# Shiakaron/Iterative-solvers-summer-2020

Hardware: AMD Instinct MI355X
Metric: Newton-steps/sec + JVP SpMV HBM GB/s (% peak), 4096^2 grid, 1/2/4/8 GPU (higher is better)
Workload: dtype f64

## Files before the change

include/nkhip.h:

```cpp
#ifndef NKHIP_H
#define NKHIP_H

#include <stdint.h>

#ifdef __cplusplus
extern "C" {
#endif

#define NK_OK 0
#define NK_NO_CONVERGENCE 1
#define NK_NONFINITE 2
#define NK_ZERO_STEP 3
#define NK_BAD_RHS 4
#define NK_EINVAL (-1)
#define NK_EHIP (-2)
#define NK_ECOMM (-3)
#define NK_ENOMEM (-4)

#define NKHIP_ABI_VERSION 3

#define NK_JVP_FD 0
#define NK_JVP_ANALYTIC 1

typedef struct nk_opts {
// ... 55 lines not shown
                int64_t ny, int64_t nx, double h, double r, double k, double g, double zs,
                double sc, void* stream);

int nk_sh_arnoldi_fused(const double* const* V_dev, const double* coef, int32_t nv,
                        const double* w_dev, double tau, const double* x0_dev, const double* G0_dev,
                        const double* z_dev, int64_t ny, int64_t nx, double h, double r, double k,
                        double g, double zs, double sc, double* v_out_dev, double* w_out_dev,
                        double* dots, void* stream);

int64_t nk_edge_elems(int64_t ny, int64_t nx);
int nk_edge_gather(const double* v_dev, double* E_dev, int64_t ny, int64_t nx, void* stream);
int nk_sh_arnoldi_fused_edges(const double* const* V_dev, const double* const* E_dev,
                              const double* coef, int32_t nv, const double* w_dev, double tau,
                              const double* x0_dev, const double* G0_dev, const double* z_dev,
                              int64_t ny, int64_t nx, double h, double r, double k, double g,
                              double zs, double sc, double* v_out_dev, double* w_out_dev,
                              double* Ev_out_dev, double* Ew_out_dev, double* dots, void* stream);
int64_t nk_arnoldi_mbox_launches(void);

int nk_dot(const double* x_dev, const double* y_dev, int64_t n, double* out, void* stream);
int nk_nrm2(const double* x_dev, int64_t n, double* out, void* stream);
int nk_maxnorm(const double* x_dev, int64_t n, double* out, void* stream);
int nk_axpy(double a, const double* x_dev, double* y_dev, int64_t n, void* stream);
int nk_scal(double a, double* x_dev, int64_t n, void* stream);
int nk_mdot(const double* const* V_dev, int32_t m, const double* w_dev, int64_t n, double* out,
            void* stream);
int nk_maxpy(const double* const* V_dev, const double* coef, int32_t m, double* y_dev, int64_t n,
             void* stream);

int nk_stream_copy(const double* src_dev, double* dst_dev, int64_t n, void* stream);

int nk_debug_bounds(int64_t* violations, int32_t* first_line, int32_t reset);
int nk_debug_mailbox(int64_t* counts, int32_t reset);
int nk_debug_ctl_step(int32_t form, int32_t t, const int32_t* ints, const double* scal,
                      const double* sig, const double* h, const double* cs, const double* sn,
                      const double* gram, const double* red, void* state_out, void* mirror_out,
                      double* prm_out, uint32_t* status_out);

int nk_comm_unique_id_bytes(void);
int nk_comm_get_unique_id(void* out);
int nk_comm_create_rccl(nk_comm** out, const void* unique_id, int32_t rank, int32_t nranks);
int nk_comm_create_loopback(nk_comm** out, int32_t nranks);
int nk_comm_peer_handle_bytes(void);
int nk_comm_create_peer(nk_comm** out, int32_t rank, int32_t nranks, int64_t max_nx,
                        void* handle_out);
int nk_comm_peer_connect(nk_comm* c, const void* handles);
int nk_comm_destroy(nk_comm* c);
int nk_comm_abort(nk_comm* c);
int nk_comm_selftest(nk_comm* c, int64_t nx, void* stream);
int nk_comm_selftest_push(nk_comm* c, int64_t nx, void* stream);

int nk_sh_create(nk_sh** out, int64_t ny_local, int64_t nx, int64_t ny_global, double h, double r,
                 double k, double g, const nk_opts* opts, nk_comm* comm, void* stream);
int nk_sh_destroy(nk_sh* s);
int nk_sh_step(nk_sh* s, const double* u_prev_dev, double* u_next_dev, nk_stats* stats);
int nk_sh_set_opts(nk_sh* s, const nk_opts* opts);
int nk_sh_kernel_profile(nk_sh* s, nk_kprof* out, int32_t max);
int nk_sh_reset_profile(nk_sh* s);
int nk_sh_step_log(nk_sh* s, double* steps, int32_t max);
int64_t nk_sh_workspace_bytes(nk_sh* s);

typedef int (*nk_residual_fn)(void* ctx, const double* x_dev, double* f_dev, int64_t n);
int64_t nk_solve_workspace_bytes(int64_t n, const nk_opts* opts);
int nk_solve(nk_residual_fn F, void* ctx, const double* x0_dev, double* x_dev, int64_t n,
             const nk_opts* opts, nk_stats* stats, void* stream, void* workspace,
             int64_t workspace_bytes);
// ... 64 lines not shown
```

iterative-solvers-summer-2020_amd/csrc/capi.cpp:

```cpp
#include <hip/hip_runtime.h>

#include <cmath>
#include <cstdlib>
#include <cstdio>
#include <cstring>
#include <mutex>
#include <memory>
#include <new>
#include <vector>

#include "../../include/nkhip.h"
#include "comm.h"
#include "nk_kernels.h"
#include "nk_solver.h"
#include "droplet_problem.h"
#include "mems_problem.h"
#include "sh_problem.h"
#include "shlin.h"

using namespace nk;

namespace {

hipStream_t S(void* s) { return static_cast<hipStream_t>(s); }
// ... 305 lines not shown
  const int rc = reduce_call(n, nv, nv, nv, res, S(stream), [&](double* part, int64_t* nb) {
    return mdot_launch(w, nullptr, P, m, n, part, S(stream), nb);
  });
  for (int i = 0; i < m; ++i) out[i] = res[i];
  return rc;
}

int nk_maxpy(const double* const* V, const double* coef, int32_t m, double* y, int64_t n,
             void* stream) {
  if (!V || !coef || !y || m < 0 || m > kMaxVec || n < 0) return NK_EINVAL;
  VecList P;
  for (int i = 0; i < m; ++i) {
    P.p[i] = V[i];
    P.c[i] = coef[i];
  }
  int64_t nb = 0;
  return hip_rc(combo_launch(y, y, 1.0, P, m, n, nullptr, S(stream), &nb));
}

int nk_stream_copy(const double* src, double* dst, int64_t n, void* stream) {
  if (!src || !dst || n < 0) return NK_EINVAL;
  return hip_rc(stream_copy_launch(src, dst, n, S(stream)));
}

int nk_debug_bounds(int64_t* violations, int32_t* first_line, int32_t reset) {
  const int rc = arnoldi_check_counters(violations, first_line, reset != 0);
  return rc == 0 ? NK_OK : (rc == -1 ? NK_EINVAL : NK_EHIP);
}

int nk_debug_mailbox(int64_t* counts, int32_t reset) {
  if (!counts) return NK_EINVAL;
  const int rc = arnoldi_mailbox_counters(counts, reset != 0);
  return rc == 0 ? NK_OK : (rc == -1 ? NK_EINVAL : NK_EHIP);
}

int nk_debug_ctl_step(int32_t form, int32_t t, const int32_t* ints, const double* scal,
                      const double* sig, const double* h, const double* cs, const double* sn,
                      const double* gram, const double* red, void* state_out, void* mirror_out,
                      double* prm_out, uint32_t* status_out) {
  if (!state_out) return int(sizeof(ArnCtlState));
  if ((form != 0 && form != 1) || t < 1 || t + 1 > kArnMaxNV || !ints || !scal || !sig || !h ||
      !cs || !sn || !gram || !red || !mirror_out || !prm_out || !status_out)
    return NK_EINVAL;
  const int nval = 2 * (t + 1) + 1;
  ArnCtlState *hS = nullptr, *dS = nullptr;
  uint32_t* status = nullptr;
  double *prm = nullptr, *dred = nullptr;
  hipError_t e = hipHostMalloc(reinterpret_cast<void**>(&hS), sizeof(ArnCtlState), 0);
  if (e == hipSuccess)
    e = hipHostMalloc(reinterpret_cast<void**>(&status), sizeof(uint32_t) * (kMaxVec + 2), 0);
  if (e == hipSuccess) e = hipMalloc(reinterpret_cast<void**>(&dS), sizeof(ArnCtlState));
  if (e == hipSuccess) e = hipMalloc(reinterpret_cast<void**>(&prm), sizeof(double) * kCtlPrm);
  if (e == hipSuccess) e = hipMalloc(reinterpret_cast<void**>(&dred), sizeof(double) * 2 * nval);
  if (e == hipSuccess) {
    std::memset(hS, 0, sizeof(ArnCtlState));
    std::memset(status, 0, sizeof(uint32_t) * (kMaxVec + 2));
    ArnCtlState& S = *hS;
    S.j = ints[0];
    S.hn_pending = ints[1];
    S.m = ints[2];
    S.nv_max = ints[3];
    S.halt = ints[4];
    S.steps = ints[5];
    S.wnorm[t - 1] = scal[0];
    S.gv[t - 1] = scal[1];
    S.sig_est[t] = scal[2];
// ... 508 lines not shown
```

iterative-solvers-summer-2020_amd/csrc/krylov.hip:

```cpp
#include <cmath>
#include <cstdlib>

#include "nk_device.h"
#include "nk_kernels.h"

namespace nk {
namespace {

constexpr int BS = kKrylovBlock;
constexpr int PAIRS = kKrylovPerThread / 2;

template <bool VEC>
__device__ __forceinline__ double2 ld2(const double* p, int64_t i, int64_t n) {
  if (VEC && i + 1 < n) return *reinterpret_cast<const double2*>(p + i);
  double2 r;
  r.x = (i < n) ? p[i] : 0.0;
  r.y = (i + 1 < n) ? p[i + 1] : 0.0;
  return r;
}

typedef double dv2 __attribute__((ext_vector_type(2)));
template <bool VEC, bool NT>
__device__ __forceinline__ double2 ld2s(const double* p, int64_t i, int64_t n) {
  if (NT && VEC && i + 1 < n) {
// ... 149 lines not shown
    if (eo.E) {
      const uint32_t nx = uint32_t(eo.nx), ny = uint32_t(eo.ny);
      uint32_t q = uint32_t(base) / nx, c = uint32_t(base) - q * nx;
#pragma unroll
      for (int k = 0; k < PAIRS; ++k) {
        if (base + k * 2 * BS < n) {
          const dv2 ev = {acc[k].x, acc[k].y};
          if (c % kEdgeW == 0)
            reinterpret_cast<dv2*>(eo.E)[2 * ((c / kEdgeW) * ny + q) + 1] = ev;
          if ((c + 2) % kEdgeW == 0 || c + 2 == nx)
            reinterpret_cast<dv2*>(eo.E)[2 * ((c + 2 == nx ? 0 : (c + 2) / kEdgeW) * ny + q)] = ev;
        }
        for (c += 2 * BS; c >= nx; c -= nx) ++q;
      }
    }
#pragma unroll
    for (int k = 0; k < PAIRS; ++k) {
      st2<VEC>(out, base + k * 2 * BS, n, acc[k]);
      const int64_t i = base + k * 2 * BS;
      if (i < n) {
        red[0] += acc[k].x * acc[k].x;
        red[1] = nmax(red[1], fabs(acc[k].x));
      }
      if (i + 1 < n) {
        red[0] += acc[k].y * acc[k].y;
        red[1] = nmax(red[1], fabs(acc[k].y));
      }
    }
  }
  if (partial) {
    const double v = block_reduce<2, 1, BS>(red);
    if (threadIdx.x < 2) partial[int64_t(threadIdx.x) * nblk + grp] = v;
  }
}

constexpr int RB = 1024;

__global__ void __launch_bounds__(RB) reduce_final_kernel(const double* partial, int64_t nblk,
                                                          int nsum, double* result,
                                                          double* result_host) {
  const int k = blockIdx.x;
  const double s = reduce_column<RB>(partial + int64_t(k) * nblk, nblk, k < nsum);
  if (threadIdx.x == 0) {
    result[k] = s;
    if (result_host) result_host[k] = s;
  }
}

template <bool VEC>
__global__ void __launch_bounds__(256) axpby_kernel(double a, const double* x, double b,
                                                    const double* y, double* out, int64_t n) {
  const int64_t i = 2 * (int64_t(blockIdx.x) * 256 + threadIdx.x);
  if (i >= n) return;
  const double2 xv = ld2<VEC>(x, i, n);
  double2 r = make_double2(a * xv.x, a * xv.y);
  if (y) {
    const double2 yv = ld2<VEC>(y, i, n);
    r.x += b * yv.x;
    r.y += b * yv.y;
  }
  st2<VEC>(out, i, n, r);
}

__global__ void __launch_bounds__(256) fddiff_kernel(double* w, const double* f0, double sc,
                                                     int64_t n) {
  const int64_t i = int64_t(blockIdx.x) * 256 + threadIdx.x;
// ... 100 lines not shown
  if (nb <= kSmallChunks) {
    if (vec)
      hipLaunchKernelGGL((combo_kernel<true, false, 8>), grid, block, 0, s, out, in, cin, P, np, n,
                         cpb, partial, rev, prm, eo);
    else
      hipLaunchKernelGGL((combo_kernel<false, false, 8>), grid, block, 0, s, out, in, cin, P, np,
                         n, cpb, partial, rev, prm, eo);
  } else if (vec && nt) {
    hipLaunchKernelGGL((combo_kernel<true, true, 2>), grid, block, 0, s, out, in, cin, P, np, n,
                       cpb, partial, rev, prm, eo);
  } else if (vec) {
    hipLaunchKernelGGL((combo_kernel<true, false, 2>), grid, block, 0, s, out, in, cin, P, np, n,
                       cpb, partial, rev, prm, eo);
  } else {
    hipLaunchKernelGGL((combo_kernel<false, false, 2>), grid, block, 0, s, out, in, cin, P, np, n,
                       cpb, partial, rev, prm, eo);
  }
  return hipGetLastError();
}
}

hipError_t combo_launch(double* out, const double* in, double cin, const VecList& P, int np,
                        int64_t n, double* partial, hipStream_t s, int64_t* nblk,
                        const EdgeOut& eo) {
  return combo_any(out, in, cin, P, np, n, partial, s, nblk, nullptr, eo);
}

hipError_t combo_prm_launch(double* out, const double* in, const double* prm, const VecList& P,
                            int np, int64_t n, hipStream_t s) {
  if (!prm || np > kArnMaxNV) return hipErrorInvalidValue;
  return combo_any(out, in, 0.0, P, np, n, nullptr, s, nullptr, prm, EdgeOut{});
}

hipError_t reduce_final_launch(const double* partial, int64_t nblk, int nsum, int nv,
                               double* result, double* result_host, hipStream_t s) {
  if (nv <= 0) return hipSuccess;
  hipLaunchKernelGGL(reduce_final_kernel, dim3(unsigned(nv)), dim3(RB), 0, s, partial, nblk, nsum,
                     result, result_host);
  return hipGetLastError();
}

namespace {
typedef double sdv2 __attribute__((ext_vector_type(2)));
__global__ void __launch_bounds__(256) stream_copy_kernel(const sdv2* __restrict__ src,
                                                          sdv2* __restrict__ dst, int64_t n2) {
  const int64_t base = int64_t(blockIdx.x) * 1024 + threadIdx.x;
  sdv2 v[4];
#pragma unroll
  for (int k = 0; k < 4; ++k) {
    const int64_t i = base + k * 256;
    if (i < n2) v[k] = __builtin_nontemporal_load(src + i);
  }
#pragma unroll
  for (int k = 0; k < 4; ++k) {
    const int64_t i = base + k * 256;
    if (i < n2) __builtin_nontemporal_store(v[k], dst + i);
  }
}

}

hipError_t stream_copy_launch(const double* src, double* dst, int64_t n, hipStream_t s) {
  if (n <= 0) return hipSuccess;
  if (!al16(src) || !al16(dst) || n % 2) return hipErrorInvalidValue;
  const int64_t n2 = n / 2;
  hipLaunchKernelGGL(stream_copy_kernel, dim3(unsigned((n2 + 1023) / 1024)), dim3(256), 0, s,
// ... 49 lines not shown
```

iterative-solvers-summer-2020_amd/csrc/lgmres.cpp:

```cpp
#include <algorithm>
#include <atomic>
#include <cstddef>
#include <cfloat>
#include <cmath>
#include <cstdlib>
#include <cstring>

#include "nk_solver.h"
#include "peer_dev.h"

namespace nk {

namespace {
constexpr double kEps = DBL_EPSILON;
constexpr double kLagMinRatio2 = 1e-12;

bool devctl_enabled(bool multi) {
  const char* v = std::getenv("NKHIP_DEVCTL");
  if (v && v[0] == '0') return false;
  if (v && v[0] == '1') return true;
  return multi;
}

bool lag_enabled() {
  static const bool on = [] {
    const char* v = std::getenv("NKHIP_LAGNORM");
    return !(v && v[0] == '0');
  }();
  return on;
}
}

int NewtonKrylov::issue_step(int j, const double* z, double zs, double znorm, bool dev_scale,
                             bool have_w) {
  const int64_t n = E_.n;
  zp_[j] = z;
  hS_->zs[j] = zs;
  double* w = V_[j + 1];
  int rc;
  if (have_w) {
    rc = NK_OK;
    st_->njvp += 1;
  } else if (dev_scale) {
    rc = P_.jvp_dev(X_, G0_, z, E_.dres(Engine::kSlotCombo), omega_, w);
    st_->njvp += 1;
  } else if (znorm == 0.0) {
    rc = E_.launch(K_COPY, 8.0 * n,
                   [&] { return hipMemsetAsync(w, 0, sizeof(double) * n, E_.s); });
    if (!rc) rc = P_.publish_edges(w);
  } else {
    rc = P_.jvp(X_, G0_, z, zs, omega_ / znorm, w);
    st_->njvp += 1;
  }
  if (rc) return rc;
  st_->n_arnoldi += 1;
  VecList P;
  for (int i = 0; i <= j; ++i) P.p[i] = V_[i];
  int64_t nblk = 0;
  const double* g = (j > 0) ? V_[j] : nullptr;
  rc = E_.launch(K_MDOT, 8.0 * n * (j + 2),
                 [&] { return mdot_launch(w, g, P, j + 1, n, E_.partial(), E_.s, &nblk); });
  if (rc) return rc;
// ... 23 lines not shown
  ArnCtlState& S = *hS_;
  S.m = m;
  S.halt = 0;
  S.steps = 0;
  S.ptol = ptol;
  S.omega = omega_;
  S.lag_ratio2 = kLagMinRatio2;
  double* const sig = S.sig;
  double* const rn = S.rn;
  double* const sig_est = S.sig_est;
  double* const wnorm = S.wnorm;
  double* const zs_ = S.zs;
  double* const h = S.h;
  sig[0] = 1.0 / b_norm;
  rn[0] = b_norm;
  double hcur[kMaxVec + 2];
  double red[2 * kMaxVec + 2];
  for (int i = 0; i < kMaxVec + 2; ++i) S.gv[i] = 0.0;
  S.gv[0] = 1.0;

  auto input = [&](int j, const double** z, double* zs, double* zn) {
    if (j < n_o) {
      const int slot = (ohead_ + j) % K;
      *z = outer_[slot];
      *zs = osig_[slot];
      *zn = osig_[slot] * orn_[slot];
    } else {
      *z = V_[j > n_o ? j : 0];
      const int q = j > n_o ? j : 0;
      *zs = sig[q];
      *zn = sig[q] * rn[q];
    }
  };
  auto finish = [&](int i, double hn) -> bool {
    for (int k = 0; k <= i; ++k) hcur[k] = h[k];
    hcur[i + 1] = hn;
    const double alpha = 1.0 / hn;
    sig[i + 1] = std::isfinite(alpha) ? alpha : 1.0;
    rn[i + 1] = hn;
    const bool breakdown = !(hn > kEps * wnorm[i]);
    for (int k = 0; k < i; ++k) {
      const double t = S.cs[k] * hcur[k] + S.sn[k] * hcur[k + 1];
      hcur[k + 1] = -S.sn[k] * hcur[k] + S.cs[k] * hcur[k + 1];
      hcur[k] = t;
    }
    detail::givens(hcur[i], hcur[i + 1], &S.cs[i], &S.sn[i]);
    hcur[i] = S.cs[i] * hcur[i] + S.sn[i] * hcur[i + 1];
    for (int k = 0; k <= i; ++k) S.R[k][i] = hcur[k];
    S.gv[i + 1] = -S.sn[i] * S.gv[i];
    S.gv[i] = S.cs[i] * S.gv[i];
    return std::fabs(S.gv[i + 1]) < ptol || breakdown;
  };

  int rc;
  {
    const double* z;
    double zs, zn;
    input(0, &z, &zs, &zn);
    const bool have = spec_.valid && n_o > 0 && z == spec_.z && zs == spec_.zs &&
                      zn == spec_.zn && V_[1] == spec_.w && X_ == spec_.x && G0_ == spec_.g;
    spec_.valid = false;
    rc = issue_step(0, z, zs, zn, false, have);
  }
  sig_est[0] = 0.0;
  if (!rc) rc = E_.sync();
  if (rc) return rc;
  int j = 0, last = 0;
  bool hn_pending = false;
  for (;;) {
    const int np = j + 1;
    std::memcpy(red, E_.hres(Engine::slot_mdot(j)), sizeof(double) * (2 * np + 1));
    double tau = 1.0;
    if (hn_pending) {
      hn_pending = false;
      if (finish(j - 1, std::sqrt(red[np + j]))) {
        st_->njvp -= 1;
        st_->n_arnoldi -= 1;
        last = j - 1;
        break;
      }
      if (sig_est[j] > 0.0) {
        tau = sig[j] / sig_est[j];
        zs_[j] = sig[j];
      }
    }
    const double ww = tau * tau * red[2 * np];
    if (!std::isfinite(ww)) return NK_NONFINITE;
    wnorm[j] = std::sqrt(ww);
    for (int i = 0; i < j; ++i) S.gram[j][i] = sig[j] * sig[i] * red[np + i];
    double hh = 0.0;
    for (int i = 0; i <= j; ++i) {
      double acc = tau * sig[i] * red[i];
      for (int k = 0; k < i; ++k) acc -= S.gram[i][k] * h[k];
      h[i] = acc;
      hh += acc * acc;
    }
    VecList U;
    for (int i = 0; i <= j; ++i) {
      U.p[i] = V_[i];
      U.c[i] = -h[i] * sig[i];
    }
    double* w = V_[j + 1];
    const bool more = j + 1 < m;
    const bool next_is_v = more && (j + 1 > n_o);
    const double est = ww - hh;
    const bool lag_step = more && lag && (!next_is_v || est > kLagMinRatio2 * ww);
    int64_t nblk = 0;
    if (lag_step && P_.has_fused(j + 1)) {
      const double* z = nullptr;
      double zs, zn;
      if (next_is_v) {
        const double e = std::sqrt(est);
        zs = 1.0 / e;
        zn = zs * e;
      } else {
        input(j + 1, &z, &zs, &zn);
      }
      if (zn != 0.0) {
        const double* Vp[kMaxVec];
        double cc[kMaxVec];
        for (int i = 0; i <= j; ++i) {
          Vp[i] = V_[i];
          cc[i] = U.c[i];
        }
        int64_t nw = 0;
        double* vout = Sv_;
        rc = P_.fused_step(Vp, cc, j + 1, w, tau, X_, G0_, z, zs, omega_ / zn, vout, V_[j + 2],
                           &nw, nullptr);
        if (rc) return rc;
        Sv_ = V_[j + 1];
        V_[j + 1] = vout;
        zp_[j + 1] = next_is_v ? vout : z;
        zs_[j + 1] = zs;
        sig_est[j + 1] = next_is_v ? zs : 0.0;
        st_->njvp += 1;
        st_->n_arnoldi += 1;
        const int np1 = j + 2;
        rc = E_.reduce_async(nw, 2 * np1 + 1, 2 * np1 + 1, Engine::slot_mdot(j + 1));
        if (rc) return rc;
        hn_pending = true;
// ... 62 lines not shown
    rc = E_.sync();
    if (rc) return rc;
    const bool stop = finish(j, std::sqrt(E_.hres(Engine::kSlotCombo)[0]));
    if (spec) zs_[j + 1] = sig[j + 1];
    if (stop || !more) {
      if (spec) {
        st_->njvp -= 1;
        st_->n_arnoldi -= 1;
      }
      last = j;
      break;
    }
    if (!spec) {
      const double* z;
      double zs, zn;
      input(j + 1, &z, &zs, &zn);
      rc = issue_step(j + 1, z, zs, zn, false);
      if (!rc) rc = E_.sync();
      if (rc) return rc;
    }
    sig_est[j + 1] = 0.0;
    ++j;
  }
  j = last;
  if (!std::isfinite(S.R[j][j])) return NK_OK;
  double y[kMaxVec + 1];
  detail::lstsq_upper(S.R, j + 1, S.gv, y);
  for (int i = 0; i <= j; ++i) {
    y[i] *= b_norm;
    if (!std::isfinite(y[i])) return NK_OK;
  }
  const int slot = (o_.outer_k > 0 && ocount_ < o_.outer_k) ? (ohead_ + ocount_) % K : ohead_;
  VecList Z;
  for (int i = 0; i <= j; ++i) {
    Z.p[i] = zp_[i];
    Z.c[i] = y[i] * zs_[i];
  }
  int64_t nblk = 0;
  double* d = outer_[slot];
  const EdgeOut eo = P_.edge_out(d);
  rc = E_.launch(K_COMBO, 8.0 * n * (j + 2), [&] {
    return combo_launch(d, nullptr, 0.0, Z, j + 1, n, E_.partial(), E_.s, &nblk, eo);
  });
  if (!rc) rc = P_.publish_edges(d, eo.E != nullptr);
  if (rc) return rc;
  double r2[2];
  rc = E_.reduce(nblk, 1, 2, r2);
  if (rc) return rc;
  const double nx = std::sqrt(r2[0]);
  if (nx > 0 && o_.outer_k > 0) {
    osig_[slot] = 1.0 / nx;
    orn_[slot] = nx;
    if (ocount_ < o_.outer_k)
      ++ocount_;
    else
      ohead_ = (ohead_ + 1) % K;
  }
  *dnorm = nx;
  *dmax = r2[1];
  *dvec = d;
  return NK_OK;
}

int NewtonKrylov::device_steps() {
  ArnCtlState& S = *hS_;
  const int t0 = S.j;
  int nvmax = t0;
  while (nvmax + 1 < S.m && nvmax + 1 <= kArnMaxNV &&
         (P_.has_fused(nvmax + 1) || P_.has_jvp_prm()))
    ++nvmax;
  if (nvmax < t0 + 1) return E_.wait_results(Engine::slot_mdot(t0), 2 * (t0 + 1) + 1);
  S.nv_max = nvmax;
  S.halt = 0;
  S.steps = 0;
  S.arrive = 0;
// ... 159 lines not shown
```

iterative-solvers-summer-2020_amd/csrc/nk_kernels.h:

```cpp
#pragma once

#include <hip/hip_runtime.h>

#include <cstdint>

#include "peer_dev.h"

struct nk_comm;

namespace nk {

bool peer_fuse_enabled();
bool slab_x_enabled(const nk_comm* c);
uint64_t device_wait_ticks();
double device_wait_seconds();

struct Field {
  const double* base;
  const double* lo;
  const double* hi;
};

inline Field periodic(const double* p) { return Field{p, nullptr, nullptr}; }

// ... 44 lines not shown
  bool nt_p0 = false;
};

bool traversal_reverse();

hipError_t stencil_launch(SMode m, const StencilArgs& a, hipStream_t s, int64_t* nblk);
int64_t stencil_partial_slots(int64_t ny, int64_t nx);
double stencil_bytes_per_point(SMode m, bool has_xt);

constexpr int kMaxVec = 64;
struct VecList {
  const double* p[kMaxVec];
  double c[kMaxVec];
};

constexpr int kKrylovBlock = 256;
constexpr int kKrylovPerThread = 8;
constexpr int64_t kKrylovChunk = int64_t(kKrylovBlock) * kKrylovPerThread;

inline int64_t krylov_blocks(int64_t n) { return (n + kKrylovChunk - 1) / kKrylovChunk; }
int64_t krylov_grid(int64_t n, int* cpb, int64_t target_blocks);

hipError_t mdot_launch(const double* a, const double* g, const VecList& P, int np, int64_t n,
                       double* partial, hipStream_t s, int64_t* nblk);
struct EdgeOut {
  double* E = nullptr;
  int64_t nx = 0, ny = 0;
};
hipError_t combo_launch(double* out, const double* in, double cin, const VecList& P, int np,
                        int64_t n, double* partial, hipStream_t s, int64_t* nblk,
                        const EdgeOut& eo = EdgeOut{});
hipError_t combo_prm_launch(double* out, const double* in, const double* prm, const VecList& P,
                            int np, int64_t n, hipStream_t s);
hipError_t reduce_final_launch(const double* partial, int64_t nblk, int nsum, int nv,
                               double* result, double* result_host, hipStream_t s);
hipError_t fddiff_launch(double* w, const double* f0, double sc, int64_t n, hipStream_t s);
hipError_t cg_update_launch(double* x, double* r, const double* p, const double* q, double alpha,
                            int64_t n, double* partial, hipStream_t s, int64_t* nblk);
hipError_t shlin_diag_launch(const double* U, const double* Uo, double k, double g, double* d,
                             int64_t n, hipStream_t s);
hipError_t stream_copy_launch(const double* src, double* dst, int64_t n, hipStream_t s);
hipError_t axpby_launch(double a, const double* x, double b, const double* y, double* out,
                        int64_t n, hipStream_t s);

constexpr int kArnMaxNV = 35;
constexpr int kEdgeW = 256;
__host__ __device__ inline int64_t edge_groups(int64_t nx) { return (nx + kEdgeW - 1) / kEdgeW; }
__host__ __device__ inline int64_t edge_elems(int64_t ny, int64_t nx) { return edge_groups(nx) * ny * 4; }
hipError_t edge_gather_launch(const double* v, double* E, int64_t ny, int64_t nx, hipStream_t s);
struct SlabX {
  char* me = nullptr;
  char* prev = nullptr;
  char* next = nullptr;
  int P = 0;
  int64_t max_nx = 0;
  uint64_t tag = 0;
  int* err = nullptr;
  uint64_t wait_ticks = 0;
};
struct ArnCtlState;
struct ArnTail {
  ArnCtlState* S = nullptr;
  ArnCtlState* H = nullptr;
  double* result = nullptr;
  double* result_host = nullptr;
  double* prm = nullptr;
// ... 97 lines not shown
```

iterative-solvers-summer-2020_amd/csrc/nk_solver.cpp:

```cpp
#include "nk_solver.h"

#include <algorithm>
#include <atomic>
#include <cfloat>
#include <cmath>
#include <cstdio>
#include <cstdlib>
#include <cstring>
#include <mutex>

namespace nk {

namespace {
constexpr double kEps = DBL_EPSILON;
constexpr int kReduceSlots = Engine::kSlots;
}

const char* kind_name(int kind) {
  static const char* names[K_NKINDS] = {"sh_fdjvp", "sh_ajvp", "sh_trial", "sh_bold",
                                         "krylov_mdot", "krylov_combo", "reduce_final", "copy",
                                         "halo", "user_F", "axpby", "arnoldi_fused",
                                         "arnoldi_edge", "edge_gather", "arnoldi_slab_edges",
                                         "arnoldi_ctl", "halo_push"};
  return (kind >= 0 && kind < K_NKINDS) ? names[kind] : "?";
// ... 320 lines not shown
    for (int k = 0; k < nv; ++k) h[k] = kUnset;
    std::atomic_thread_fence(std::memory_order_release);
  }
  int rc = launch(K_REDUCE, 8.0 * nblk * nv, [&] {
    return reduce_final_launch(partial_, nblk, nsum, nv, dres_ + slot,
                               multi ? nullptr : hres_ + slot, s);
  });
  if (rc || !multi) return rc;
  if (!host_copy) return comm->allreduce(dres_ + slot, nsum, nv, s);
  return comm->allreduce_host(dres_ + slot, hres_ + slot, nsum, nv, s);
}

int Engine::reduce(int64_t nblk, int nsum, int nv, double* out) {
  int rc = reduce_async(nblk, nsum, nv, kSlotSync);
  if (!rc) rc = sync();
  if (rc) return rc;
  std::memcpy(out, hres_ + kSlotSync, sizeof(double) * nv);
  return NK_OK;
}

namespace detail {

void givens(double a, double b, double* c, double* s) {
  if (b == 0.0) {
    *c = 1.0;
    *s = 0.0;
    return;
  }
  const double r = std::hypot(a, b);
  *c = a / r;
  *s = b / r;
}

void lstsq_upper(const double (*R)[kMaxVec + 1], int n, const double* g, double* y) {
  double dmax = 0.0, dmin = INFINITY;
  for (int i = 0; i < n; ++i) {
    dmax = std::max(dmax, std::fabs(R[i][i]));
    dmin = std::min(dmin, std::fabs(R[i][i]));
  }
  if (n > 0 && dmin > kEps * n * dmax) {
    for (int i = n - 1; i >= 0; --i) {
      double acc = g[i];
      for (int k = i + 1; k < n; ++k) acc -= R[i][k] * y[k];
      y[i] = acc / R[i][i];
    }
    return;
  }
  std::vector<double> A(n * n), Vm(n * n, 0.0);
  for (int i = 0; i < n; ++i)
    for (int k = 0; k < n; ++k) A[i * n + k] = (k >= i) ? R[i][k] : 0.0;
  for (int i = 0; i < n; ++i) Vm[i * n + i] = 1.0;
  for (int sweep = 0; sweep < 60; ++sweep) {
    double off = 0.0;
    for (int p = 0; p < n - 1; ++p)
      for (int q = p + 1; q < n; ++q) {
        double a = 0, b = 0, c = 0;
        for (int i = 0; i < n; ++i) {
          a += A[i * n + p] * A[i * n + p];
          b += A[i * n + q] * A[i * n + q];
          c += A[i * n + p] * A[i * n + q];
        }
        if (c == 0.0) continue;
        off = std::max(off, std::fabs(c) / std::sqrt(a * b + 1e-300));
        const double zeta = (b - a) / (2.0 * c);
        const double t = std::copysign(1.0, zeta) / (std::fabs(zeta) + std::sqrt(1.0 + zeta * zeta));
        const double cs = 1.0 / std::sqrt(1.0 + t * t), sn = cs * t;
        for (int i = 0; i < n; ++i) {
          const double ap = A[i * n + p], aq = A[i * n + q];
          A[i * n + p] = cs * ap - sn * aq;
          A[i * n + q] = sn * ap + cs * aq;
          const double vp = Vm[i * n + p], vq = Vm[i * n + q];
          Vm[i * n + p] = cs * vp - sn * vq;
          Vm[i * n + q] = sn * vp + cs * vq;
// ... 261 lines not shown
```

iterative-solvers-summer-2020_amd/csrc/nk_solver.h:

```cpp
#pragma once

#include <hip/hip_runtime.h>

#include <cstdint>
#include <string>
#include <vector>

#include "../../include/nkhip.h"
#include "comm.h"
#include "nk_kernels.h"

namespace nk {

enum Kind : int {
  K_FDJVP = 0,
  K_AJVP,
  K_TRIAL,
  K_BOLD,
  K_MDOT,
  K_COMBO,
  K_REDUCE,
  K_COPY,
  K_HALO,
  K_USERF,
// ... 205 lines not shown
  Engine& E_;
  Problem& P_;
  nk_opts o_;
  int init_status_ = NK_OK;
  double *X_ = nullptr, *Xt_ = nullptr, *Fx_ = nullptr, *Ft_ = nullptr, *G0_ = nullptr,
         *Gt_ = nullptr;
  double* Sv_ = nullptr;
  std::vector<double*> V_;
  std::vector<double*> outer_;
  std::vector<double> osig_, orn_;
  int ocount_ = 0, ohead_ = 0;
  double omega_ = 0.0;
  double* d_ = nullptr;
  nk_stats* st_ = nullptr;
  std::vector<double> steps_;
  double fx_norm_ = 0.0;
  double rdiff_ = 0.0;
  double f_tol_ = 0.0;
  struct {
    bool valid = false;
    const double* z = nullptr;
    double zs = 0.0, zn = 0.0;
    double* w = nullptr;
    const double* x = nullptr;
    const double* g = nullptr;
  } spec_;
};

nk_opts default_opts();

namespace detail {
void givens(double a, double b, double* c, double* s);
void lstsq_upper(const double (*R)[kMaxVec + 1], int n, const double* g, double* y);
}

}
```

iterative-solvers-summer-2020_amd/nkhip/_lib.py:

```python
from __future__ import annotations

import ctypes as C
import os

import torch

LIB_PATH = os.path.join(os.path.dirname(os.path.abspath(__file__)), "libnkhip.so")
LIB_PATH = os.environ.get("NKHIP_LIB") or LIB_PATH

NK_OK = 0
NK_NO_CONVERGENCE = 1
NK_NONFINITE = 2
NK_ZERO_STEP = 3
NK_BAD_RHS = 4
NK_EINVAL = -1
NK_EHIP = -2
NK_ECOMM = -3
NK_ENOMEM = -4
ABI_VERSION = 3
NK_JVP_FD = 0
NK_JVP_ANALYTIC = 1


class nk_opts(C.Structure):
# ... 40 lines not shown
_D = C.c_double
_I64 = C.c_int64
_I32 = C.c_int32

SIGNATURES = [
    ("nk_version", C.c_char_p, []),
    ("nk_abi_version", C.c_int, []),
    ("nk_opts_default", C.c_int, [C.POINTER(nk_opts)]),
    ("nk_status_string", C.c_char_p, [C.c_int]),
    ("nk_lap5_apply", C.c_int, [_P, _P, _I64, _I64, _D, _P]),
    ("nk_sh13_apply", C.c_int, [_P, _P, _I64, _I64, _D, _D, _P]),
    ("nk_sh_residual", C.c_int, [_P, _P, _P, _I64, _I64, _D, _D, _D, _D, _P]),
    ("nk_sh_jvp", C.c_int, [_P, _P, _P, _I64, _I64, _D, _D, _D, _D, _P]),
    ("nk_sh_fdjvp", C.c_int, [_P, _P, _P, _P, _I64, _I64, _D, _D, _D, _D, _D, _D, _P]),
    ("nk_sh_arnoldi_fused", C.c_int, [C.POINTER(_P), C.POINTER(_D), _I32, _P, _D, _P, _P, _P,
                                      _I64, _I64, _D, _D, _D, _D, _D, _D, _P, _P,
                                      C.POINTER(_D), _P]),
    ("nk_edge_elems", C.c_int64, [_I64, _I64]),
    ("nk_arnoldi_mbox_launches", C.c_int64, []),
    ("nk_edge_gather", C.c_int, [_P, _P, _I64, _I64, _P]),
    ("nk_sh_arnoldi_fused_edges", C.c_int, [C.POINTER(_P), C.POINTER(_P), C.POINTER(_D), _I32,
                                            _P, _D, _P, _P, _P, _I64, _I64, _D, _D, _D, _D, _D,
                                            _D, _P, _P, _P, _P, C.POINTER(_D), _P]),
    ("nk_dot", C.c_int, [_P, _P, _I64, C.POINTER(_D), _P]),
    ("nk_nrm2", C.c_int, [_P, _I64, C.POINTER(_D), _P]),
    ("nk_maxnorm", C.c_int, [_P, _I64, C.POINTER(_D), _P]),
    ("nk_axpy", C.c_int, [_D, _P, _P, _I64, _P]),
    ("nk_scal", C.c_int, [_D, _P, _I64, _P]),
    ("nk_mdot", C.c_int, [C.POINTER(_P), _I32, _P, _I64, C.POINTER(_D), _P]),
    ("nk_maxpy", C.c_int, [C.POINTER(_P), C.POINTER(_D), _I32, _P, _I64, _P]),
    ("nk_stream_copy", C.c_int, [_P, _P, _I64, _P]),
    ("nk_debug_bounds", C.c_int, [C.POINTER(_I64), C.POINTER(_I32), _I32]),
    ("nk_debug_mailbox", C.c_int, [C.POINTER(_I64), _I32]),
    ("nk_debug_ctl_step", C.c_int, [_I32, _I32, _P, _P, _P, _P, _P, _P, _P, _P, _P, _P, _P, _P]),
    ("nk_comm_unique_id_bytes", C.c_int, []),
    ("nk_comm_get_unique_id", C.c_int, [_P]),
    ("nk_comm_create_rccl", C.c_int, [C.POINTER(_P), _P, _I32, _I32]),
    ("nk_comm_create_loopback", C.c_int, [C.POINTER(_P), _I32]),
    ("nk_comm_peer_handle_bytes", C.c_int, []),
    ("nk_comm_create_peer", C.c_int, [C.POINTER(_P), _I32, _I32, _I64, _P]),
    ("nk_comm_peer_connect", C.c_int, [_P, _P]),
    ("nk_comm_destroy", C.c_int, [_P]),
    ("nk_comm_abort", C.c_int, [_P]),
    ("nk_comm_selftest", C.c_int, [_P, _I64, _P]),
    ("nk_comm_selftest_push", C.c_int, [_P, _I64, _P]),
    ("nk_sh_create", C.c_int, [C.POINTER(_P), _I64, _I64, _I64, _D, _D, _D, _D,
                               C.POINTER(nk_opts), _P, _P]),
    ("nk_sh_destroy", C.c_int, [_P]),
    ("nk_sh_step", C.c_int, [_P, _P, _P, C.POINTER(nk_stats)]),
    ("nk_sh_set_opts", C.c_int, [_P, C.POINTER(nk_opts)]),
    ("nk_sh_kernel_profile", C.c_int, [_P, C.POINTER(nk_kprof), _I32]),
    ("nk_sh_reset_profile", C.c_int, [_P]),
    ("nk_sh_step_log", C.c_int, [_P, C.POINTER(_D), _I32]),
    ("nk_sh_workspace_bytes", C.c_int64, [_P]),
    ("nk_solve_workspace_bytes", C.c_int64, [_I64, C.POINTER(nk_opts)]),
    ("nk_solve", C.c_int, [RESIDUAL_FN, _P, _P, _P, _I64, C.POINTER(nk_opts),
                           C.POINTER(nk_stats), _P, _P, _I64]),
    ("nk_drop_params_default", C.c_int, [C.POINTER(nk_drop_params)]),
    ("nk_drop_create", C.c_int, [C.POINTER(_P), C.POINTER(nk_drop_params), C.POINTER(nk_opts),
                                 _P]),
    ("nk_drop_destroy", C.c_int, [_P]),
    ("nk_drop_set_state", C.c_int, [_P, _P, _P]),
    ("nk_drop_get_state", C.c_int, [_P, _P, _P]),
    ("nk_drop_step", C.c_int, [_P, _D, _D, _I32, C.POINTER(nk_stats), C.POINTER(_D),
                               C.POINTER(_D)]),
    ("nk_drop_set_scale", C.c_int, [_P, _D]),
# ... 61 lines not shown
```

iterative-solvers-summer-2020_amd/nkhip/ops.py:

```python
from __future__ import annotations

import ctypes as C

import torch

from ._lib import check, lib


def _stream():
    return C.c_void_p(torch.cuda.current_stream().cuda_stream)


def _dev(t: torch.Tensor, name: str) -> torch.Tensor:
    if not isinstance(t, torch.Tensor) or not t.is_cuda:
        raise TypeError(f"{name} must be a CUDA (HIP) tensor")
    if t.dtype != torch.float64:
        raise TypeError(f"{name} must be float64 (the reference computes in fp64)")
    if not t.is_contiguous():
        raise ValueError(f"{name} must be contiguous")
    return t


def _ptr(t: torch.Tensor):
    return C.c_void_p(t.data_ptr())
# ... 120 lines not shown


def axpy(a, x, y):
    _dev(x, "x")
    _dev(y, "y")
    check(lib.nk_axpy(float(a), _ptr(x), _ptr(y), x.numel(), _stream()), "nk_axpy")
    return y


def scal(a, x):
    _dev(x, "x")
    check(lib.nk_scal(float(a), _ptr(x), x.numel(), _stream()), "nk_scal")
    return x


def mdot(V, w):
    _dev(w, "w")
    m = len(V)
    ptrs = (C.c_void_p * max(m, 1))(*[_dev(v, "V[i]").data_ptr() for v in V])
    out = (C.c_double * max(m, 1))()
    check(lib.nk_mdot(ptrs, m, _ptr(w), w.numel(), out, _stream()), "nk_mdot")
    return [out[i] for i in range(m)]


def maxpy(V, coef, y):
    _dev(y, "y")
    m = len(V)
    ptrs = (C.c_void_p * max(m, 1))(*[_dev(v, "V[i]").data_ptr() for v in V])
    cs = (C.c_double * max(m, 1))(*[float(c) for c in coef])
    check(lib.nk_maxpy(ptrs, cs, m, _ptr(y), y.numel(), _stream()), "nk_maxpy")
    return y


def stream_copy(src, out=None):
    src = _dev(src, "src")
    out = torch.empty_like(src) if out is None else _dev(out, "out")
    if out.numel() != src.numel():
        raise ValueError("stream_copy: size mismatch")
    check(lib.nk_stream_copy(_ptr(src), _ptr(out), src.numel(), _stream()), "nk_stream_copy")
    return out
```

Measured before the change: 29.04.

## Predict LGMRES convergence and close the solve with a fused three-output combo kernel

```diff
diff --git a/include/nkhip.h b/include/nkhip.h
--- a/include/nkhip.h
+++ b/include/nkhip.h
@@ -111,6 +111,9 @@
 
 int nk_debug_bounds(int64_t* violations, int32_t* first_line, int32_t reset);
 int nk_debug_mailbox(int64_t* counts, int32_t reset);
+int nk_debug_close(const double* const* P_dev, const double* cN, const double* cA,
+                   const double* cB, int32_t m, int64_t n, double* A_dev, double* B_dev,
+                   double* norm2, void* stream);
 int nk_debug_ctl_step(int32_t form, int32_t t, const int32_t* ints, const double* scal,
                       const double* sig, const double* h, const double* cs, const double* sn,
                       const double* gram, const double* red, void* state_out, void* mirror_out,
diff --git a/iterative-solvers-summer-2020_amd/csrc/capi.cpp b/iterative-solvers-summer-2020_amd/csrc/capi.cpp
--- a/iterative-solvers-summer-2020_amd/csrc/capi.cpp
+++ b/iterative-solvers-summer-2020_amd/csrc/capi.cpp
@@ -361,6 +361,25 @@
   if (!counts) return NK_EINVAL;
   const int rc = arnoldi_mailbox_counters(counts, reset != 0);
   return rc == 0 ? NK_OK : (rc == -1 ? NK_EINVAL : NK_EHIP);
+}
+
+int nk_debug_close(const double* const* P, const double* cN, const double* cA, const double* cB,
+                   int32_t m, int64_t n, double* A, double* B, double* norm2, void* stream) {
+  if (!P || !cN || !cA || !cB || !A || !B || A == B || !norm2 || m < 1 || m > kMaxVec || n < 1)
+    return NK_EINVAL;
+  CloseList L;
+  for (int i = 0; i < m; ++i) {
+    for (int k = 0; k < i; ++k)
+      if (P[k] == P[i]) return NK_EINVAL;
+    if (!P[i]) return NK_EINVAL;
+    L.p[i] = P[i];
+    L.cN[i] = cN[i];
+    L.cA[i] = cA[i];
+    L.cB[i] = cB[i];
+  }
+  return reduce_call(n, 1, 1, 1, norm2, S(stream), [&](double* part, int64_t* nb) {
+    return close_launch(A, B, L, m, n, part, S(stream), nb);
+  });
 }
 
 int nk_debug_ctl_step(int32_t form, int32_t t, const int32_t* ints, const double* scal,
diff --git a/iterative-solvers-summer-2020_amd/csrc/krylov.hip b/iterative-solvers-summer-2020_amd/csrc/krylov.hip
--- a/iterative-solvers-summer-2020_amd/csrc/krylov.hip
+++ b/iterative-solvers-summer-2020_amd/csrc/krylov.hip
@@ -205,6 +205,72 @@
     const double v = block_reduce<2, 1, BS>(red);
     if (threadIdx.x < 2) partial[int64_t(threadIdx.x) * nblk + grp] = v;
   }
+}
+
+struct Close {};
+template <class Tag, bool VEC, bool NT, int UNR>
+__global__ void __launch_bounds__(BS) combo_kernel(double* outA, double* outB, CloseList P, int np,
+                                                   int64_t n, int cpb, double* partial, bool rev) {
+  const int64_t nblk = gridDim.x;
+  const int64_t bid = blockIdx.x;
+  double red[1] = {0.0};
+  const int64_t grp = rev ? nblk - 1 - bid : bid;
+  for (int cc = 0; cc < cpb; ++cc) {
+    const int64_t chunk = grp * cpb + cc;
+    if (chunk * kKrylovChunk >= n) break;
+    const int64_t base = chunk * kKrylovChunk + 2 * int64_t(threadIdx.x);
+    double2 aN[PAIRS], aA[PAIRS], aB[PAIRS];
+#pragma unroll
+    for (int k = 0; k < PAIRS; ++k) aN[k] = aA[k] = aB[k] = make_double2(0.0, 0.0);
+    int i = 0;
+    for (; i + UNR <= np; i += UNR) {
+      double2 pv[UNR][PAIRS];
+#pragma unroll
+      for (int u = 0; u < UNR; ++u) {
+#pragma unroll
+        for (int k = 0; k < PAIRS; ++k) pv[u][k] = ld2s<VEC, NT>(P.p[i + u], base + k * 2 * BS, n);
+      }
+#pragma unroll
+      for (int u = 0; u < UNR; ++u) {
+        const double cn = P.cN[i + u], ca = P.cA[i + u], cb = P.cB[i + u];
+#pragma unroll
+        for (int k = 0; k < PAIRS; ++k) {
+          aN[k].x += cn * pv[u][k].x;
+          aN[k].y += cn * pv[u][k].y;
+          aA[k].x += ca * pv[u][k].x;
+          aA[k].y += ca * pv[u][k].y;
+          aB[k].x += cb * pv[u][k].x;
+          aB[k].y += cb * pv[u][k].y;
+        }
+      }
+    }
+    for (; i < np; ++i) {
+      const double* p = P.p[i];
+      const double cn = P.cN[i], ca = P.cA[i], cb = P.cB[i];
+      double2 pv[PAIRS];
+#pragma unroll
+      for (int k = 0; k < PAIRS; ++k) pv[k] = ld2s<VEC, NT>(p, base + k * 2 * BS, n);
+#pragma unroll
+      for (int k = 0; k < PAIRS; ++k) {
+        aN[k].x += cn * pv[k].x;
+        aN[k].y += cn * pv[k].y;
+        aA[k].x += ca * pv[k].x;
+        aA[k].y += ca * pv[k].y;
+        aB[k].x += cb * pv[k].x;
+        aB[k].y += cb * pv[k].y;
+      }
+    }
+#pragma unroll
+    for (int k = 0; k < PAIRS; ++k) {
+      st2<VEC>(outA, base + k * 2 * BS, n, aA[k]);
+      st2<VEC>(outB, base + k * 2 * BS, n, aB[k]);
+      const int64_t e = base + k * 2 * BS;
+      if (e < n) red[0] += aN[k].x * aN[k].x;
+      if (e + 1 < n) red[0] += aN[k].y * aN[k].y;
+    }
+  }
+  const double v = block_reduce<1, 1, BS>(red);
+  if (threadIdx.x == 0) partial[grp] = v;
 }
 
 constexpr int RB = 1024;
@@ -371,6 +437,40 @@
   return combo_any(out, in, 0.0, P, np, n, nullptr, s, nullptr, prm, EdgeOut{});
 }
 
+hipError_t close_launch(double* outA, double* outB, const CloseList& P, int np, int64_t n,
+                        double* partial, hipStream_t s, int64_t* nblk) {
+  if (np < 1 || np > kMaxVec || !outA || !outB || outA == outB || !partial)
+    return hipErrorInvalidValue;
+  static const int target = env_int("NKHIP_COMBO_BLOCKS", 1 << 30);
+  int cpb = 0;
+  const int64_t nb = krylov_grid(n, &cpb, target);
+  if (nblk) *nblk = nb;
+  if (nb == 0) return hipSuccess;
+  bool vec = al16(outA) && al16(outB);
+  for (int i = 0; i < np; ++i) vec = vec && al16(P.p[i]);
+  const bool rev = traversal_reverse();
+  static const bool nt = env_int("NKHIP_NT", 1) != 0;
+  const dim3 grid{unsigned(nb)}, block{unsigned(BS)};
+  if (nb <= kSmallChunks) {
+    if (vec)
+      hipLaunchKernelGGL((combo_kernel<Close, true, false, 8>), grid, block, 0, s, outA, outB, P,
+                         np, n, cpb, partial, rev);
+    else
+      hipLaunchKernelGGL((combo_kernel<Close, false, false, 8>), grid, block, 0, s, outA, outB, P,
+                         np, n, cpb, partial, rev);
+  } else if (vec && nt) {
+    hipLaunchKernelGGL((combo_kernel<Close, true, true, 2>), grid, block, 0, s, outA, outB, P, np,
+                       n, cpb, partial, rev);
+  } else if (vec) {
+    hipLaunchKernelGGL((combo_kernel<Close, true, false, 2>), grid, block, 0, s, outA, outB, P, np,
+                       n, cpb, partial, rev);
+  } else {
+    hipLaunchKernelGGL((combo_kernel<Close, false, false, 2>), grid, block, 0, s, outA, outB, P,
+                       np, n, cpb, partial, rev);
+  }
+  return hipGetLastError();
+}
+
 hipError_t reduce_final_launch(const double* partial, int64_t nblk, int nsum, int nv,
                                double* result, double* result_host, hipStream_t s) {
   if (nv <= 0) return hipSuccess;
diff --git a/iterative-solvers-summer-2020_amd/csrc/lgmres.cpp b/iterative-solvers-summer-2020_amd/csrc/lgmres.cpp
--- a/iterative-solvers-summer-2020_amd/csrc/lgmres.cpp
+++ b/iterative-solvers-summer-2020_amd/csrc/lgmres.cpp
@@ -28,6 +28,13 @@
     return !(v && v[0] == '0');
   }();
   return on;
+}
+
+int close_mode_env() {
+  const char* v = std::getenv("NKHIP_CLOSE");
+  if (v && v[0] == '0') return 0;
+  if (v && v[0] == '2') return 2;
+  return 1;
 }
 }
 
@@ -117,18 +124,27 @@
       *zn = sig[q] * rn[q];
     }
   };
+  auto rotated = [&](int i, double hn, double* hc) {
+    for (int k = 0; k <= i; ++k) hc[k] = h[k];
+    hc[i + 1] = hn;
+    for (int k = 0; k < i; ++k) {
+      const double t = S.cs[k] * hc[k] + S.sn[k] * hc[k + 1];
+      hc[k + 1] = -S.sn[k] * hc[k] + S.cs[k] * hc[k + 1];
+      hc[k] = t;
+    }
+  };
+  auto would_stop = [&](int i, double hn) -> bool {
+    double hc[kMaxVec + 2], c, s;
+    rotated(i, hn, hc);
+    detail::givens(hc[i], hc[i + 1], &c, &s);
+    return std::fabs(-s * S.gv[i]) < ptol || !(hn > kEps * wnorm[i]);
+  };
   auto finish = [&](int i, double hn) -> bool {
-    for (int k = 0; k <= i; ++k) hcur[k] = h[k];
-    hcur[i + 1] = hn;
+    rotated(i, hn, hcur);
     const double alpha = 1.0 / hn;
     sig[i + 1] = std::isfinite(alpha) ? alpha : 1.0;
     rn[i + 1] = hn;
     const bool breakdown = !(hn > kEps * wnorm[i]);
-    for (int k = 0; k < i; ++k) {
-      const double t = S.cs[k] * hcur[k] + S.sn[k] * hcur[k + 1];
-      hcur[k + 1] = -S.sn[k] * hcur[k] + S.cs[k] * hcur[k + 1];
-      hcur[k] = t;
-    }
     detail::givens(hcur[i], hcur[i + 1], &S.cs[i], &S.sn[i]);
     hcur[i] = S.cs[i] * hcur[i] + S.sn[i] * hcur[i + 1];
     for (int k = 0; k <= i; ++k) S.R[k][i] = hcur[k];
@@ -151,6 +167,8 @@
   if (!rc) rc = E_.sync();
   if (rc) return rc;
   int j = 0, last = 0;
+  int close_mode = lag ? close_mode_env() : 0;
+  bool closed = false;
   bool hn_pending = false;
   for (;;) {
     const int np = j + 1;
@@ -189,8 +207,79 @@
     const bool more = j + 1 < m;
     const bool next_is_v = more && (j + 1 > n_o);
     const double est = ww - hh;
-    const bool lag_step = more && lag && (!next_is_v || est > kLagMinRatio2 * ww);
     int64_t nblk = 0;
+    bool predicted = false;
+    if (close_mode && P_.has_fused(j + 1) && j + 2 < int(V_.size())) {
+      const double hn_est = std::sqrt(est);
+      if (close_mode == 2) {
+        predicted = true;
+        close_mode = 1;
+      } else if (hn_est > kEps * wnorm[j]) {
+        predicted = !more || (est > kLagMinRatio2 * ww && would_stop(j, hn_est));
+      }
+    }
+    if (predicted) {
+      double hc[kMaxVec + 2], a[kMaxVec + 1], b[kMaxVec + 1];
+      rotated(j, 0.0, hc);
+      if (j > 0 && !detail::lstsq_upper_direct(S.R, j)) {
+        close_mode = 0;
+        predicted = false;
+      }
+      for (int i = j - 1; predicted && i >= 0; --i) {
+        double accA = S.gv[i], accB = hc[i];
+        for (int k = i + 1; k < j; ++k) {
+          accA -= S.R[i][k] * a[k];
+          accB -= S.R[i][k] * b[k];
+        }
+        a[i] = accA / S.R[i][i];
+        b[i] = accB / S.R[i][i];
+      }
+      CloseList C;
+      int nc = 0;
+      auto entry = [&](const double* p) -> int {
+        for (int q = 0; q < nc; ++q)
+          if (C.p[q] == p) return q;
+        if (nc == kMaxVec) return -1;
+        C.p[nc] = p;
+        C.cN[nc] = C.cA[nc] = C.cB[nc] = 0.0;
+        return nc++;
+      };
+      if (predicted) {
+        C.cN[entry(w)] = tau;
+        for (int i = 0; i <= j; ++i) C.cN[entry(V_[i])] = U.c[i];
+        for (int i = 0; i <= j; ++i) {
+          const int q = entry(zp_[i]);
+          if (q < 0) {
+            predicted = false;
+            break;
+          }
+          if (i < j) {
+            C.cA[q] += b_norm * a[i] * zs_[i];
+            C.cB[q] -= b[i] * zs_[i];
+          } else {
+            C.cB[q] += zs_[j];
+          }
+        }
+      }
+      if (predicted) {
+        rc = E_.launch(K_COMBO, 8.0 * n * (nc + 2), [&] {
+          return close_launch(Sv_, V_[j + 2], C, nc, n, E_.partial(), E_.s, &nblk);
+        });
+        if (rc) return rc;
+        double v2 = 0.0;
+        rc = E_.reduce(nblk, 1, 1, &v2);
+        if (rc) return rc;
+        const double hn = std::sqrt(v2);
+        if (!more || would_stop(j, hn)) {
+          finish(j, hn);
+          last = j;
+          closed = true;
+          break;
+        }
+      }
+    }
+    const bool lag_step =
+        more && lag && !predicted && (!next_is_v || est > kLagMinRatio2 * ww);
     if (lag_step && P_.has_fused(j + 1)) {
       const double* z = nullptr;
       double zs, zn;
@@ -319,15 +408,24 @@
   }
   const int slot = (o_.outer_k > 0 && ocount_ < o_.outer_k) ? (ohead_ + ocount_) % K : ohead_;
   VecList Z;
-  for (int i = 0; i <= j; ++i) {
-    Z.p[i] = zp_[i];
-    Z.c[i] = y[i] * zs_[i];
+  int nz = j + 1;
+  if (closed && detail::lstsq_upper_direct(S.R, j + 1)) {
+    nz = 2;
+    Z.p[0] = Sv_;
+    Z.c[0] = 1.0;
+    Z.p[1] = V_[j + 2];
+    Z.c[1] = y[j];
+  } else {
+    for (int i = 0; i <= j; ++i) {
+      Z.p[i] = zp_[i];
+      Z.c[i] = y[i] * zs_[i];
+    }
   }
   int64_t nblk = 0;
   double* d = outer_[slot];
   const EdgeOut eo = P_.edge_out(d);
-  rc = E_.launch(K_COMBO, 8.0 * n * (j + 2), [&] {
-    return combo_launch(d, nullptr, 0.0, Z, j + 1, n, E_.partial(), E_.s, &nblk, eo);
+  rc = E_.launch(K_COMBO, 8.0 * n * (nz + 1), [&] {
+    return combo_launch(d, nullptr, 0.0, Z, nz, n, E_.partial(), E_.s, &nblk, eo);
   });
   if (!rc) rc = P_.publish_edges(d, eo.E != nullptr);
   if (rc) return rc;
diff --git a/iterative-solvers-summer-2020_amd/csrc/nk_kernels.h b/iterative-solvers-summer-2020_amd/csrc/nk_kernels.h
--- a/iterative-solvers-summer-2020_amd/csrc/nk_kernels.h
+++ b/iterative-solvers-summer-2020_amd/csrc/nk_kernels.h
@@ -100,6 +100,12 @@
                         const EdgeOut& eo = EdgeOut{});
 hipError_t combo_prm_launch(double* out, const double* in, const double* prm, const VecList& P,
                             int np, int64_t n, hipStream_t s);
+struct CloseList {
+  const double* p[kMaxVec];
+  double cN[kMaxVec], cA[kMaxVec], cB[kMaxVec];
+};
+hipError_t close_launch(double* outA, double* outB, const CloseList& P, int np, int64_t n,
+                        double* partial, hipStream_t s, int64_t* nblk);
 hipError_t reduce_final_launch(const double* partial, int64_t nblk, int nsum, int nv,
                                double* result, double* result_host, hipStream_t s);
 hipError_t fddiff_launch(double* w, const double* f0, double sc, int64_t n, hipStream_t s);
diff --git a/iterative-solvers-summer-2020_amd/csrc/nk_solver.cpp b/iterative-solvers-summer-2020_amd/csrc/nk_solver.cpp
--- a/iterative-solvers-summer-2020_amd/csrc/nk_solver.cpp
+++ b/iterative-solvers-summer-2020_amd/csrc/nk_solver.cpp
@@ -376,13 +376,17 @@
   *s = b / r;
 }
 
-void lstsq_upper(const double (*R)[kMaxVec + 1], int n, const double* g, double* y) {
+bool lstsq_upper_direct(const double (*R)[kMaxVec + 1], int n) {
   double dmax = 0.0, dmin = INFINITY;
   for (int i = 0; i < n; ++i) {
     dmax = std::max(dmax, std::fabs(R[i][i]));
     dmin = std::min(dmin, std::fabs(R[i][i]));
   }
-  if (n > 0 && dmin > kEps * n * dmax) {
+  return n > 0 && dmin > kEps * n * dmax;
+}
+
+void lstsq_upper(const double (*R)[kMaxVec + 1], int n, const double* g, double* y) {
+  if (lstsq_upper_direct(R, n)) {
     for (int i = n - 1; i >= 0; --i) {
       double acc = g[i];
       for (int k = i + 1; k < n; ++k) acc -= R[i][k] * y[k];
diff --git a/iterative-solvers-summer-2020_amd/csrc/nk_solver.h b/iterative-solvers-summer-2020_amd/csrc/nk_solver.h
--- a/iterative-solvers-summer-2020_amd/csrc/nk_solver.h
+++ b/iterative-solvers-summer-2020_amd/csrc/nk_solver.h
@@ -261,6 +261,7 @@
 namespace detail {
 void givens(double a, double b, double* c, double* s);
 void lstsq_upper(const double (*R)[kMaxVec + 1], int n, const double* g, double* y);
+bool lstsq_upper_direct(const double (*R)[kMaxVec + 1], int n);
 }
 
 }
diff --git a/iterative-solvers-summer-2020_amd/nkhip/_lib.py b/iterative-solvers-summer-2020_amd/nkhip/_lib.py
--- a/iterative-solvers-summer-2020_amd/nkhip/_lib.py
+++ b/iterative-solvers-summer-2020_amd/nkhip/_lib.py
@@ -96,6 +96,8 @@
     ("nk_stream_copy", C.c_int, [_P, _P, _I64, _P]),
     ("nk_debug_bounds", C.c_int, [C.POINTER(_I64), C.POINTER(_I32), _I32]),
     ("nk_debug_mailbox", C.c_int, [C.POINTER(_I64), _I32]),
+    ("nk_debug_close", C.c_int, [C.POINTER(_P), C.POINTER(_D), C.POINTER(_D), C.POINTER(_D), _I32,
+                                 _I64, _P, _P, C.POINTER(_D), _P]),
     ("nk_debug_ctl_step", C.c_int, [_I32, _I32, _P, _P, _P, _P, _P, _P, _P, _P, _P, _P, _P, _P]),
     ("nk_comm_unique_id_bytes", C.c_int, []),
     ("nk_comm_get_unique_id", C.c_int, [_P]),
diff --git a/iterative-solvers-summer-2020_amd/nkhip/ops.py b/iterative-solvers-summer-2020_amd/nkhip/ops.py
--- a/iterative-solvers-summer-2020_amd/nkhip/ops.py
+++ b/iterative-solvers-summer-2020_amd/nkhip/ops.py
@@ -176,6 +176,28 @@
     return y
 
 
+def lgmres_close(P, cN, cA, cB, A=None, B=None):
+    m = len(P)
+    if m < 1 or not (len(cN) == len(cA) == len(cB) == m):
+        raise ValueError("lgmres_close: one (cN, cA, cB) triple per vector, at least one vector")
+    for i, p in enumerate(P):
+        _dev(p, "P[i]")
+        if p.numel() != P[0].numel():
+            raise ValueError("lgmres_close: size mismatch")
+    if len({p.data_ptr() for p in P}) != m:
+        raise ValueError("lgmres_close: the vectors must be distinct (one list entry per tensor)")
+    A = torch.empty_like(P[0]) if A is None else _dev(A, "A")
+    B = torch.empty_like(P[0]) if B is None else _dev(B, "B")
+    if A.numel() != P[0].numel() or B.numel() != P[0].numel():
+        raise ValueError("lgmres_close: size mismatch")
+    ptrs = (C.c_void_p * m)(*[p.data_ptr() for p in P])
+    arr = [(C.c_double * m)(*[float(c) for c in cs]) for cs in (cN, cA, cB)]
+    r = C.c_double()
+    check(lib.nk_debug_close(ptrs, *arr, m, P[0].numel(), _ptr(A), _ptr(B), C.byref(r),
+                             _stream()), "nk_debug_close")
+    return A, B, r.value
+
+
 def stream_copy(src, out=None):
     src = _dev(src, "src")
     out = torch.empty_like(src) if out is None else _dev(out, "out")
```

Result: faster. 30.02, median of 6 (+3.4%).
